# zju3dv/PVO

Hardware: AMD Instinct MI355X
Metric: VO keyframe updates/sec (8-keyframe window, 512x384, 36 edges; 6 graph updates + edge rebuild per keyframe) (higher is better)
Workload: dtype f16 (volume, lookup, update operator) / f32 (BA assembly) / f64 (pose solve); 1 GPU; S-B: BASELINE.json configs[1] window (8 keyframes, 48x64 maps, E=36, itrs=2), synthetic; edges=36, parallelism=independent window per GPU

## Files before the change

### pvo_amd/csrc/ba.hip

```cpp
#include "se3.h"
#include "conv1x1_tile.h"
#include "glo_tile.h"
#include <stdlib.h>
#include <type_traits>

namespace {

constexpr float kMinDepth = 0.25f;

constexpr double kFix = 268435456.0, kInvFix = 1.0 / 268435456.0;
__device__ __forceinline__ void fix_add(long long* sys, long long idx, double v, int* meta) {
  if (!(fabs(v) < 3.0e10)) { meta[4] = 1; return; }
#ifdef PVO_BA_NO_ATOMICS
  if (idx >= 0) return;
#endif
  atomicAdd(reinterpret_cast<unsigned long long*>(sys + idx), static_cast<unsigned long long>(__double2ll_rn(v * kFix)));
}
constexpr int kDealEdges = 2;
constexpr int kPPT = 2;
constexpr int kChunkA = 256 * kPPT;
constexpr int kMaxSep = 12;
constexpr int kXchgDoubles = 2 + 36 * kMaxSep * kMaxSep + 12 * kMaxSep;


// ... 2365 lines not shown
        const int ta0 = on0 ? 16 * tti[K] + lc - c0 : 0, tb0 = on0 ? 16 * ttj[K] + lc - c0 : 0;
        const int ta1 = on1 ? 16 * tti[K1] + lc - c0 : 0, tb1 = on1 ? 16 * ttj[K1] + lc - c0 : 0;
        double a00 = pan[dense_swz(ta0, lr)], b00 = pan[dense_swz(tb0, lr)], a01 = pan[dense_swz(ta0, 4 + lr)], b01 = pan[dense_swz(tb0, 4 + lr)];
        double a10 = pan[dense_swz(ta1, lr)], b10 = pan[dense_swz(tb1, lr)], a11 = pan[dense_swz(ta1, 4 + lr)], b11 = pan[dense_swz(tb1, 4 + lr)];
        if (!on0) { a00 = 0.0; a01 = 0.0; }
        if (!on1) { a10 = 0.0; a11 = 0.0; }
        C[K] = __builtin_amdgcn_mfma_f64_16x16x4f64(-a00, b00, C[K], 0, 0, 0);
        if (K + 1 < SLOTS) C[K1] = __builtin_amdgcn_mfma_f64_16x16x4f64(-a10, b10, C[K1], 0, 0, 0);
        C[K] = __builtin_amdgcn_mfma_f64_16x16x4f64(-a01, b01, C[K], 0, 0, 0);
        if (K + 1 < SLOTS) C[K1] = __builtin_amdgcn_mfma_f64_16x16x4f64(-a11, b11, C[K1], 0, 0, 0);
      };
      switch (u0 >> 1) {
#define PVO_DENSE_PAIR(K) case K / 2: if (K < SLOTS) { if (K >= nsl) break; pair(std::integral_constant<int, (K < SLOTS ? K : 0)>{}); } [[fallthrough]];
        PVO_DENSE_PAIR(0) PVO_DENSE_PAIR(2) PVO_DENSE_PAIR(4) PVO_DENSE_PAIR(6) PVO_DENSE_PAIR(8) PVO_DENSE_PAIR(10) PVO_DENSE_PAIR(12)
        PVO_DENSE_PAIR(14) PVO_DENSE_PAIR(16)
#undef PVO_DENSE_PAIR
        default: break;
      }
    }
    DENSE_STEP_PROBE(11);
    if (kb8 + 1 < nb) extract(kb8 + 1);
    DENSE_STEP_PROBE(12);
    DENSE_STEP_PROBE(13);
    __syncthreads();
    DENSE_STEP_PROBE(14);
  }
  BA_PROBE(2);

  if (wave == 0) {
    double z[3];
#pragma unroll
    for (int m = 0; m < 3; ++m) {
      const int c = lane + 64 * m;
      z[m] = c < n ? Lp[8 * dense_panel_off(c >> 3, N) + dense_swz(n - 8 * (c >> 3), c & 7)] : 0.0;
    }
    for (int kb8 = nb - 1; kb8 >= 0; --kb8) {
      const int c0 = 8 * kb8, m0 = c0 >> 6, l0 = c0 & 63;
      const int nv = (n - c0 < 8) ? n - c0 : 8;
      const double* pan = Lp + 8 * dense_panel_off(kb8, N);
      double Lk[28], rdv[8];
#pragma unroll
      for (int j = 0; j < 8; ++j) {
        rdv[j] = rdg[c0 + j];
#pragma unroll
        for (int i = j + 1; i < 8; ++i) Lk[i * (i - 1) / 2 + j] = pan[dense_swz(i, j)];
      }
      const double zsel = m0 == 0 ? z[0] : (m0 == 1 ? z[1] : z[2]);
      double x[8];
#pragma unroll
      for (int j = 0; j < 8; ++j) {
        const int lo = __builtin_amdgcn_readlane(static_cast<int>(__double_as_longlong(zsel) & 0xffffffffLL), l0 + j);
        const int hi = __builtin_amdgcn_readlane(static_cast<int>(__double_as_longlong(zsel) >> 32), l0 + j);
        x[j] = __longlong_as_double((static_cast<long long>(hi) << 32) | static_cast<unsigned int>(lo));
      }
#pragma unroll
      for (int j = 7; j >= 0; --j) {
        double v = x[j];
#pragma unroll
        for (int i = 7; i > j; --i) v -= Lk[i * (i - 1) / 2 + j] * x[i];
        x[j] = (j < nv) ? v * rdv[j] : 0.0;
      }
#pragma unroll
      for (int m = 0; m < 3; ++m) {
        const int c = lane + 64 * m;
        if (c < c0) {
          const double* pc = Lp + 8 * dense_panel_off(c >> 3, N);
          double v = z[m];
#pragma unroll
          for (int i = 0; i < 8; ++i) v -= pc[dense_swz(c0 + i - 8 * (c >> 3), c & 7)] * x[i];
          z[m] = v;
        } else if (c < c0 + 8) {
          double v = x[0];
#pragma unroll
          for (int j = 1; j < 8; ++j) v = (c - c0 == j) ? x[j] : v;
          z[m] = v;
        }
      }
    }
#pragma unroll
    for (int m = 0; m < 3; ++m) {
      const int c = lane + 64 * m;
      if (c < n) xs[c] = z[m];
    }
  }
  __syncthreads();
  BA_PROBE(4);
  solve_epilogue([&](int i) { return xs[i]; }, fail | meta[4] | meta[2], true, 0, P, t0, poses, dx_ws, dx_out, meta, status_out, true,
                 [] { BA_PROBE(5); });
}

constexpr int kNB = 48;
__global__ __launch_bounds__(256) void dense_panel_kernel(double* __restrict__ A, double* __restrict__ Ldiag, int n, int kb, int* __restrict__ meta) {
  __shared__ double Lk[kNB][kNB + 1];
  __shared__ double Xs[kNB][kNB + 1];
  __shared__ double rinv[kNB], ldg[kNB];
  const int tid = threadIdx.x;
  const int c0 = kNB * kb, nc = (n - c0 < kNB) ? n - c0 : kNB;
  const int rb = kb + blockIdx.x, r0 = kNB * rb;
  for (int t = tid; t < kNB * kNB; t += 256) {
    const int r = t / kNB, c = t - r * kNB;
    Lk[r][c] = (r < nc && c <= r) ? A[static_cast<size_t>(c0 + r) * n + c0 + c] : 0.0;
    const int rr = r0 + r;
    Xs[r][c] = (rr <= n && c < nc) ? A[static_cast<size_t>(rr) * n + c0 + c] : 0.0;
  }
  __syncthreads();
  bool ok = true;
  for (int j0 = 0; j0 < nc; j0 += 8) {
    const int nv = (nc - j0 < 8) ? nc - j0 : 8;
    double L[36], av[8];
    if (tid < 2 * kNB) {
      const bool isx = tid >= kNB;
      const int t = isx ? tid - kNB : tid;
      if (isx || (t >= j0 && t < nc)) {
        double (*Row)[kNB + 1] = isx ? Xs : Lk;
#pragma unroll
        for (int i = 0; i < 8; ++i) {
#pragma unroll
          for (int j = 0; j <= i; ++j) L[i * (i + 1) / 2 + j] = Lk[j0 + i][j0 + j];
        }
#pragma unroll
        for (int j = 0; j < 8; ++j) av[j] = Row[t][j0 + j];
      }
    }
    __syncthreads();
    if (tid < 2 * kNB) {
      const bool isx = tid >= kNB;
      const int t = isx ? tid - kNB : tid;
      if (isx || (t >= j0 && t < nc)) {
        double (*Row)[kNB + 1] = isx ? Xs : Lk;
#pragma unroll
        for (int j = 0; j < 8; ++j) {
          double d = L[j * (j + 1) / 2 + j];
#pragma unroll
          for (int k = 0; k < j; ++k) d -= L[j * (j + 1) / 2 + k] * L[j * (j + 1) / 2 + k];
          const bool real = j < nv;
          ok = ok && (!real || d > 0.0);
          const double rs = (real && ok) ? rsqrt_nr(d) : 0.0;
          if (!isx && t == j0 + j) { rinv[j0 + j] = rs; ldg[j0 + j] = d * rs; }
          L[j * (j + 1) / 2 + j] = rs;
#pragma unroll
          for (int i = j + 1; i < 8; ++i) {
            double v = L[i * (i + 1) / 2 + j];
#pragma unroll
            for (int k = 0; k < j; ++k) v -= L[i * (i + 1) / 2 + k] * L[j * (j + 1) / 2 + k];
            L[i * (i + 1) / 2 + j] = v * rs;
          }
          double v = av[j];
#pragma unroll
          for (int k = 0; k < j; ++k) v -= av[k] * L[j * (j + 1) / 2 + k];
          av[j] = v * rs;
        }
#pragma unroll
        for (int j = 0; j < 8; ++j) if (j < nv && (isx || j0 + j <= t)) Row[t][j0 + j] = av[j];
      }
    }
    __syncthreads();
    const int c1 = j0 + 8;
    if (c1 < nc) {
      const int ty = tid >> 4, tx = tid & 15;
      for (int r = c1 + ty; r < nc + kNB; r += 16) {
        const bool isx = r >= nc;
        double (*Row)[kNB + 1] = isx ? Xs : Lk;
        const int rr = isx ? r - nc : r;
        double a8[8];
#pragma unroll
        for (int k = 0; k < 8; ++k) a8[k] = Row[rr][j0 + k];
// ... 899 lines not shown
      hipLaunchKernelGGL(ba_schur_reduce_kernel, dim3(kSchurStagePairs, Kgrid), dim3(256), 0, st, w.plan, w.spart, w.srow, w.sT, sys, gx, 6 * P);
      PVO_CHECK_LAUNCH();
    }
  }
  return PVO_OK;
}

extern "C" int pvo_ba_finish(float* poses, float* disps, void* sys_,
                             const int64_t* ii, const int64_t* jj,
                             int E, int nframes, int ht, int wd, int t0, int t1,
                             float lm, float ep, int motion_only, int clamp_frames, float disp_min,
                             float* dx_out, float* dz_out, int dz_rows, int* status_out,
                             void* workspace, size_t workspace_bytes, void* stream) {
  return pvo_ba_finish_riders(poses, disps, sys_, ii, jj, E, nframes, ht, wd, t0, t1, lm, ep, motion_only, clamp_frames, disp_min,
                              dx_out, dz_out, dz_rows, status_out, workspace, workspace_bytes, nullptr, stream);
}

extern "C" int pvo_ba_finish_conv1x1(float* poses, float* disps, void* sys_,
                                     const int64_t* ii, const int64_t* jj,
                                     int E, int nframes, int ht, int wd, int t0, int t1,
                                     float lm, float ep, int motion_only, int clamp_frames, float disp_min,
                                     float* dx_out, float* dz_out, int dz_rows, int* status_out,
                                     void* workspace, size_t workspace_bytes,
                                     const void* cx, const void* cw, const float* cbias, void* cy, long long crows, int cCout, int cdtype,
                                     void* stream) {
  pvo_ba_riders r{};
  r.cx = cx; r.cw = cw; r.cbias = cbias; r.cy = cy; r.crows = crows; r.cCout = cCout; r.cdtype = cdtype;
  return pvo_ba_finish_riders(poses, disps, sys_, ii, jj, E, nframes, ht, wd, t0, t1, lm, ep, motion_only, clamp_frames, disp_min,
                              dx_out, dz_out, dz_rows, status_out, workspace, workspace_bytes, cy ? &r : nullptr, stream);
}

static int ba_finish_impl(float* poses, float* disps, void* sys_, const long long* msg, const int* first_s,
                          const int64_t* ii, const int64_t* jj,
                          int E, int nframes, int ht, int wd, int t0, int t1,
                          float lm, float ep, int motion_only, int clamp_frames, float disp_min,
                          float* dx_out, float* dz_out, int dz_rows, int* status_out,
                          void* workspace, size_t workspace_bytes,
                          const pvo_ba_riders* jobs, void* stream);

extern "C" int pvo_ba_finish_riders(float* poses, float* disps, void* sys_,
                                    const int64_t* ii, const int64_t* jj,
                                    int E, int nframes, int ht, int wd, int t0, int t1,
                                    float lm, float ep, int motion_only, int clamp_frames, float disp_min,
                                    float* dx_out, float* dz_out, int dz_rows, int* status_out,
                                    void* workspace, size_t workspace_bytes,
                                    const pvo_ba_riders* jobs, void* stream) {
  if (!sys_) return PVO_EINVAL;
  return ba_finish_impl(poses, disps, sys_, nullptr, nullptr, ii, jj, E, nframes, ht, wd, t0, t1, lm, ep, motion_only, clamp_frames, disp_min,
                        dx_out, dz_out, dz_rows, status_out, workspace, workspace_bytes, jobs, stream);
}

extern "C" size_t pvo_ba_packed_elems(const int* first_host, int P) {
  if (!first_host || P < 0) return 0;
  size_t blocks = 0;
  for (int b = 0; b < P; ++b) {
    const int f = first_host[b] < b ? (first_host[b] < 0 ? 0 : first_host[b]) : b;
    blocks += static_cast<size_t>(b - f + 1) * 36;
  }
  return blocks + static_cast<size_t>(6) * P;
}

extern "C" int pvo_ba_pack(void* sys_, const int* first_s, void* msg, int P, void* stream) {
  if (!sys_ || !first_s || !msg || P < 0) return PVO_EINVAL;
  if (P > kMaxEnvBlocks) return PVO_EUNSUPPORTED;
  if (P == 0) return PVO_OK;
  const int n6 = 6 * P;
  hipLaunchKernelGGL(ba_pack_kernel, dim3((n6 * n6 + n6 + 2047) / 2048), dim3(256), 0, pvo_stream(stream),
                     static_cast<long long*>(sys_), first_s, static_cast<long long*>(msg), n6);
  PVO_CHECK_LAUNCH();
  return PVO_OK;
}

extern "C" int pvo_ba_finish_packed(float* poses, float* disps, const void* msg, const int* first_s,
                                    const int64_t* ii, const int64_t* jj,
                                    int E, int nframes, int ht, int wd, int t0, int t1,
                                    float lm, float ep, int motion_only, int clamp_frames, float disp_min,
                                    float* dx_out, float* dz_out, int dz_rows, int* status_out,
                                    void* workspace, size_t workspace_bytes, void* stream) {
  if (!msg || !first_s) return PVO_EINVAL;
  return ba_finish_impl(poses, disps, nullptr, static_cast<const long long*>(msg), first_s, ii, jj, E, nframes, ht, wd, t0, t1, lm, ep, motion_only,
                        clamp_frames, disp_min, dx_out, dz_out, dz_rows, status_out, workspace, workspace_bytes, nullptr, stream);
}

enum SolveKind { kSolveStatus, kSolveDense, kSolveEnvelope, kSolveChain, kSolveBlocks };
struct SolveForm { SolveKind kind; int chol; };
static SolveForm solve_form(int P, int E, bool packed, int knob) {
  if (P == 0) return {kSolveStatus, 0};
  if (knob >= 1 && knob <= 3) return {kSolveChain, knob - 1};
  if (knob == 4) return {kSolveEnvelope, 2};
  if (knob == 6 && !packed) return {kSolveBlocks, 0};
  if (P <= kDenseMaxPoses) return {kSolveDense, 0};
  if (knob != 5 && !packed && static_cast<long long>(E) > 8LL * P) return {kSolveBlocks, 0};
  return {kSolveEnvelope, 2};
}

static int ba_finish_impl(float* poses, float* disps, void* sys_, const long long* msg, const int* first_s,
                          const int64_t* ii, const int64_t* jj,
                          int E, int nframes, int ht, int wd, int t0, int t1,
                          float lm, float ep, int motion_only, int clamp_frames, float disp_min,
                          float* dx_out, float* dz_out, int dz_rows, int* status_out,
                          void* workspace, size_t workspace_bytes,
                          const pvo_ba_riders* jobs, void* stream) {
  Riders rider{};
  size_t rider_lds = 0;
  if (jobs && jobs->cy && jobs->crows > 0) {
    if (!jobs->cx || !jobs->cw || jobs->cCout <= 0 || jobs->cCout % 192) return PVO_EINVAL;
    if (jobs->cdtype != PVO_F16 && jobs->cdtype != PVO_BF16) return PVO_EUNSUPPORTED;
    if (pvo_misaligned16(jobs->cx, jobs->cw, jobs->cy)) return PVO_EINVAL;
    if (jobs->crows > (1LL << 24)) return PVO_EUNSUPPORTED;
    rider.cx = static_cast<const uint16_t*>(jobs->cx); rider.cw = static_cast<const uint16_t*>(jobs->cw); rider.cbias = jobs->cbias;
    rider.cy = static_cast<uint16_t*>(jobs->cy); rider.crows = jobs->crows; rider.cCout = jobs->cCout; rider.cdtype = jobs->cdtype;
    rider.crow_blocks = static_cast<int>((jobs->crows + 63) / 64);
    rider.cblocks = rider.crow_blocks * (jobs->cCout / 192);
    rider_lds = c1t::kTileBytes;
  }
  if (jobs && jobs->gpart && jobs->gE > 0 && jobs->gHW > 0) {
    if (!jobs->gnet || !jobs->gw || jobs->gE > 65535) return PVO_EINVAL;
    if (jobs->gdtype != PVO_F16 && jobs->gdtype != PVO_BF16) return PVO_EUNSUPPORTED;
    if (pvo_misaligned16(jobs->gnet, jobs->gw)) return PVO_EINVAL;
    rider.gnet = static_cast<const uint16_t*>(jobs->gnet); rider.gw = static_cast<const uint16_t*>(jobs->gw); rider.gbias = jobs->gbias;
    rider.gpart = jobs->gpart; rider.gHW = jobs->gHW; rider.gchunks = (jobs->gHW + 255) / 256; rider.gdtype = jobs->gdtype;
    rider.gblocks = jobs->gE * rider.gchunks;
    if (rider_lds < static_cast<size_t>(glt::kTileBytes)) rider_lds = glt::kTileBytes;
  }
  if (jobs && jobs->xg && jobs->xE > 0) {
    if (!jobs->xpart || !jobs->xwt || !jobs->xbias || jobs->xchunks <= 0) return PVO_EINVAL;
    rider.xpart = jobs->xpart; rider.xwt = jobs->xwt; rider.xbias = jobs->xbias; rider.xg = jobs->xg;
    rider.xchunks = jobs->xchunks; rider.xblocks = jobs->xE;
    if (rider_lds < 512) rider_lds = 512;
  }
  const int rider_blocks = rider.cblocks + rider.gblocks + rider.xblocks;
  int rc = check_common(E, nframes, ht, wd, t0, t1);
  if (rc != PVO_OK) return rc;
  if (clamp_frames < 0 || clamp_frames > nframes) return PVO_EINVAL;
  const int P = t1 - t0, HW = ht * wd;
  long long* sys = static_cast<long long*>(sys_);
  if (!poses || !disps || (!sys && !msg) || !workspace) return PVO_EINVAL;
  if (P > kMaxEnvBlocks) return PVO_EUNSUPPORTED;
  if (workspace_bytes < pvo_ba_workspace_bytes(E, P, nframes, HW)) return PVO_EWORKSPACE;
  Ws w = carve(ws_base(workspace), E, P, nframes, HW);
  hipStream_t st = pvo_stream(stream);
  const int n6 = 6 * P;
  const SolveForm form = solve_form(P, E, msg != nullptr, pvo_knob(PVO_KNOB_BA_SOLVER));
  if (msg && form.kind == kSolveStatus) return PVO_OK;
  constexpr size_t kSolveLdsMax = 142000;
  if (form.kind == kSolveDense) {
    const size_t dl = dense_lds_bytes(n6);
    const size_t lds = dl > rider_lds ? dl : rider_lds;
    const int Td = dense_N(n6) / 16;
    if (!pvo_allow_lds<ba_solve_dense_kernel<4>>(kSolveLdsMax) || !pvo_allow_lds<ba_solve_dense_kernel<14>>(kSolveLdsMax) ||
        !pvo_allow_lds<ba_solve_dense_kernel<17>>(kSolveLdsMax))
      return PVO_ELAUNCH;
    const auto kernel = Td <= 5 ? ba_solve_dense_kernel<4> : (Td <= 10 ? ba_solve_dense_kernel<14> : ba_solve_dense_kernel<17>);
    hipLaunchKernelGGL(kernel, dim3(1 + rider_blocks), dim3(256), lds, st, sys, msg, first_s, poses, w.dx, dx_out, w.plan.meta, status_out,
                       P, t0, lm, ep, rider);
  } else if (form.kind == kSolveEnvelope || form.kind == kSolveChain) {
    int* part = form.kind == kSolveEnvelope ? reinterpret_cast<int*>(w.xchg) : nullptr;
    if (msg) {
      hipLaunchKernelGGL(ba_env_packed_kernel, dim3(P), dim3(256), 0, st, msg, first_s, w.plan.env, n6);
      hipLaunchKernelGGL(ba_prepare_packed_kernel, dim3(P + 1), dim3(256), 0, st, msg, first_s, w.chol, w.plan.env, n6, lm, ep,
                         static_cast<long long>(kSolveLdsMax), part);
    } else {
      hipLaunchKernelGGL(ba_env_kernel, dim3((n6 * n6 + 2047) / 2048), dim3(256), 0, st, sys, w.plan.env, n6);
      hipLaunchKernelGGL(ba_prepare_kernel, dim3((n6 * n6 + n6 + 2047) / 2048), dim3(256), 0, st, sys, w.chol, w.plan.env, n6, lm, ep,
                         static_cast<long long>(kSolveLdsMax), part);
    }
    PVO_CHECK_LAUNCH();
    if (!part && hipMemsetAsync(w.xchg, 0, 16, st) != hipSuccess) return PVO_ELAUNCH;
    if (!pvo_allow_lds<ba_solve_twin_kernel>(kSolveLdsMax)) return PVO_ELAUNCH;
    hipLaunchKernelGGL(ba_solve_twin_kernel, dim3(2 + rider_blocks), dim3(256), kSolveLdsMax > rider_lds ? kSolveLdsMax : rider_lds, st,
                       w.chol, poses, w.dx, dx_out, w.plan.meta, status_out, P, t0, w.plan.env, static_cast<long long>(kSolveLdsMax), w.xchg,
                       form.chol, rider);
  } else {
    if (form.kind == kSolveBlocks) {
      hipLaunchKernelGGL(ba_prepare_kernel, dim3((n6 * n6 + n6 + 2047) / 2048), dim3(256), 0, st, sys, w.chol, w.plan.env, n6, lm, ep,
                         0LL , static_cast<int*>(nullptr));
      PVO_CHECK_LAUNCH();
      if (hipMemsetAsync(w.xchg, 0, 16, st) != hipSuccess) return PVO_ELAUNCH;
      const int nkb = (n6 + kNB - 1) / kNB, nrb = (n6 + 1 + kNB - 1) / kNB;
      for (int kb = 0; kb < nkb; ++kb) {
        hipLaunchKernelGGL(dense_panel_kernel, dim3(nrb - kb), dim3(256), 0, st, w.chol, w.ldiag, n6, kb, w.plan.meta);
        const int m = nrb - kb - 1;
        if (m > 0) hipLaunchKernelGGL(dense_update_kernel, dim3(m * (m + 1) / 2), dim3(256), 0, st, w.chol, n6, kb, nrb);
      }
      PVO_CHECK_LAUNCH();
      double* yrow = w.chol + static_cast<size_t>(n6) * n6;
      for (int kb = nkb - 1; kb >= 0; --kb)
        hipLaunchKernelGGL(dense_back_kernel, dim3(kb + 1), dim3(256), 0, st, w.chol, w.ldiag, yrow, w.xvec, n6, kb);
      PVO_CHECK_LAUNCH();
    }
    if (rider_lds > 48 * 1024 && !pvo_allow_lds<dense_finish_kernel>(kSolveLdsMax)) return PVO_ELAUNCH;
    hipLaunchKernelGGL(dense_finish_kernel, dim3(1 + rider_blocks), dim3(256), rider_lds, st, w.xvec, poses, w.dx, dx_out, w.plan.meta, status_out, P, t0, rider);
  }
  PVO_CHECK_LAUNCH();
  if (!motion_only && E + P > 0) {
    const int Kmax = (nframes < P + E) ? nframes : (P + E);
    hipLaunchKernelGGL(ba_backsub_kernel, dim3((HW + 255) / 256, Kmax > clamp_frames ? Kmax : clamp_frames), dim3(256), 0, st,
                       w.plan, jj, w.Ei, w.Eij, w.Q, w.w, w.dx, disps, dz_out, dz_rows, HW, t0, P, clamp_frames, disp_min);
    PVO_CHECK_LAUNCH();
  }
  return PVO_OK;
}

extern "C" int pvo_ba_last_partition(void* workspace, size_t workspace_bytes, int E, int P, int nframes, int HW, int* out, void* stream) {
  if (!workspace || !out || E < 0 || P < 0) return PVO_EINVAL;
  if (workspace_bytes < pvo_ba_workspace_bytes(E, P, nframes, HW)) return PVO_EWORKSPACE;
  out[0] = out[1] = 0;
  const SolveKind kind = solve_form(P, E, false, pvo_knob(PVO_KNOB_BA_SOLVER)).kind;
  if (kind == kSolveStatus || kind == kSolveDense) return PVO_OK;
  Ws w = carve(ws_base(workspace), E, P, nframes, HW);
  int host[4] = {0, 0, 0, 0};
  if (hipMemcpyAsync(host, w.xchg, sizeof(host), hipMemcpyDeviceToHost, pvo_stream(stream)) != hipSuccess) return PVO_ELAUNCH;
  if (hipStreamSynchronize(pvo_stream(stream)) != hipSuccess) return PVO_ELAUNCH;
  out[0] = host[2]; out[1] = host[3];
  return PVO_OK;
}

extern "C" int pvo_ba_rig(float* poses, float* disps, const float* intrinsics,
                          const float* targets, const float* weights, const float* eta,
                          const int64_t* ii, const int64_t* jj,
                          int E, int nframes, int ht, int wd, int K_eta,
                          int t0, int t1, int iterations, float lm, float ep, int motion_only,
                          float* dx_out, float* dz_out, int dz_rows, int* status_out,
                          void* workspace, size_t workspace_bytes,
                          const float* disps_sens, float alpha, float baseline, void* stream) {
  int rc = check_common(E, nframes, ht, wd, t0, t1);
  if (rc != PVO_OK) return rc;
  if (iterations < 0) return PVO_EINVAL;
  if (disps_sens && !(alpha > 0.0f)) return PVO_EINVAL;
  if (!(baseline >= 0.0f) || !(baseline < __builtin_inff())) return PVO_EINVAL;
  const int P = t1 - t0, HW = ht * wd;
  if (!workspace) return PVO_EINVAL;
  if (workspace_bytes < pvo_ba_workspace_bytes(E, P, nframes, HW)) return PVO_EWORKSPACE;
  Ws w = carve(ws_base(workspace), E, P, nframes, HW);
  hipStream_t st = pvo_stream(stream);
  hipLaunchKernelGGL(ba_plan_kernel, dim3(1), dim3(256), 0, st, ii, jj, w.plan, E, nframes, t0, t1,
                     K_eta, motion_only, disps_sens, alpha, baseline);
  PVO_CHECK_LAUNCH();
  for (int it = 0; it < iterations; ++it) {
    rc = pvo_ba_local(poses, disps, intrinsics, targets, weights, eta, ii, jj, E, nframes, ht, wd, K_eta,
                      t0, t1, (motion_only ? 1 : 0) | (it > 0 ? 2 : 0), w.sys, workspace, workspace_bytes, stream);
    if (rc != PVO_OK) return rc;
    rc = pvo_ba_finish(poses, disps, w.sys, ii, jj, E, nframes, ht, wd, t0, t1, lm, ep, motion_only, 0, 0.0f,
                       dx_out, dz_out, dz_rows, status_out, workspace, workspace_bytes, stream);
    if (rc != PVO_OK) return rc;
  }
  return PVO_OK;
}

extern "C" int pvo_ba_prior(float* poses, float* disps, const float* intrinsics,
                            const float* targets, const float* weights, const float* eta,
                            const int64_t* ii, const int64_t* jj,
                            int E, int nframes, int ht, int wd, int K_eta,
                            int t0, int t1, int iterations, float lm, float ep, int motion_only,
                            float* dx_out, float* dz_out, int dz_rows, int* status_out,
                            void* workspace, size_t workspace_bytes,
                            const float* disps_sens, float alpha, void* stream) {
  return pvo_ba_rig(poses, disps, intrinsics, targets, weights, eta, ii, jj, E, nframes, ht, wd, K_eta, t0, t1, iterations, lm, ep,
                    motion_only, dx_out, dz_out, dz_rows, status_out, workspace, workspace_bytes, disps_sens, alpha, 0.0f, stream);
}

extern "C" int pvo_ba(float* poses, float* disps, const float* intrinsics,
                      const float* targets, const float* weights, const float* eta,
                      const int64_t* ii, const int64_t* jj,
                      int E, int nframes, int ht, int wd, int K_eta,
                      int t0, int t1, int iterations, float lm, float ep, int motion_only,
                      float* dx_out, float* dz_out, int dz_rows, int* status_out,
                      void* workspace, size_t workspace_bytes, void* stream) {
  return pvo_ba_prior(poses, disps, intrinsics, targets, weights, eta, ii, jj, E, nframes, ht, wd, K_eta, t0, t1, iterations, lm, ep,
                      motion_only, dx_out, dz_out, dz_rows, status_out, workspace, workspace_bytes, nullptr, 0.0f, stream);
}

extern "C" int pvo_ba_sigma(const void* sys_, void* workspace, size_t workspace_bytes,
                            const int64_t* ii, const int64_t* jj,
                            int E, int P, int nframes, int ht, int wd, int t0, float lm, float ep,
                            double* pose_cov, float* var_cond, float* var_pose, int* status_out, void* stream) {
  if (P < 0) return PVO_EINVAL;
  int rc = check_common(E, nframes, ht, wd, t0, t0 + P);
  if (rc != PVO_OK) return rc;
  if (P > kSigmaMaxPoses) return PVO_EUNSUPPORTED;
  if (!workspace || (P > 0 && (!sys_ || !pose_cov))) return PVO_EINVAL;
  if (E == 0 || !ii || !jj) return PVO_EINVAL;
  const int HW = ht * wd, n = 6 * P;
  if (workspace_bytes < pvo_ba_workspace_bytes(E, P, nframes, HW)) return PVO_EWORKSPACE;
  Ws w = carve(ws_base(workspace), E, P, nframes, HW);
  hipStream_t st = pvo_stream(stream);
  if (P > 0) {
    hipLaunchKernelGGL(ba_sigma_prepare_kernel, dim3((n * n + 255) / 256), dim3(256), 0, st, static_cast<const long long*>(sys_), w.chol, n, lm, ep);
    hipLaunchKernelGGL(ba_sigma_factor_kernel, dim3(1), dim3(1024), 0, st, w.chol, n, w.plan.meta, status_out);
    hipLaunchKernelGGL(ba_sigma_invtri_kernel, dim3(n), dim3(64), 0, st, w.chol, n);
    hipLaunchKernelGGL(ba_sigma_product_kernel, dim3((n + 63) / 64, n), dim3(64), 0, st, w.chol, pose_cov, n);
    PVO_CHECK_LAUNCH();
// ... 91 lines not shown
```

### pvo_amd/droid_backends.py

```python
import ctypes
import itertools

import torch

from . import _lib
from ._lib import PvoHipError, check

_DT = {torch.float32: _lib.PVO_F32, torch.float16: _lib.PVO_F16,
       torch.bfloat16: _lib.PVO_BF16, torch.float64: _lib.PVO_F64}

_ws_cache = {}


def _contig(t, name):
    if not t.is_contiguous():
        raise RuntimeError("%s must be contiguous" % name)


def _dev(*ts):
    dev = None
    for t in ts:
        if t is None:
            continue
        if not t.is_cuda:
# ... 1333 lines not shown
    stride = int(stride)
    y = torch.empty(N, Cout, (H - 1) // stride + 1, (W - 1) // stride + 1, dtype=x.dtype, device=dev)
    with torch.cuda.device(dev):
        check(_lib.load().pvo_conv1x1_planes(_ptr(x), _ptr(w), _vp(bias), _ptr(y), N, Cin, Cout, H, W, stride, _dtype_code(x, "x"), _stream(dev)), "conv1x1_planes")
    return y


def conv_planes_supported(ksize, stride, cin, cout):
    return bool(_lib.load().pvo_conv_planes_supported(int(ksize), int(stride), int(cin), int(cout)))


class PackedConvFilter:
    __slots__ = ("frag", "ksize", "cin", "cout", "dtype")

    def __init__(self, frag, ksize, cin, cout, dtype):
        self.frag, self.ksize, self.cin, self.cout, self.dtype = frag, ksize, cin, cout, dtype


def conv_planes_pack(weight):
    dev = _dev(weight)
    if weight.dim() != 4 or weight.shape[2] != weight.shape[3] or weight.dtype not in (torch.float16, torch.bfloat16) or not weight.is_contiguous():
        raise PvoHipError("conv_planes_pack: weight must be a contiguous 16-bit [Cout,Cin,k,k] tensor")
    Cout, Cin, k, _ = weight.shape
    lib = _lib.load()
    nbytes = lib.pvo_conv_planes_filter_bytes(k, Cin, Cout)
    if nbytes == 0:
        raise PvoHipError("conv_planes_pack: unsupported filter %d x %d, %d -> %d channels" % (k, k, Cin, Cout))
    frag = torch.empty(nbytes // 2, dtype=weight.dtype, device=dev)
    with torch.cuda.device(dev):
        check(lib.pvo_conv_planes_pack(_ptr(weight), _ptr(frag), k, Cin, Cout, _dtype_code(weight, "weight"), _stream(dev)), "conv_planes_pack")
    return PackedConvFilter(frag, k, Cin, Cout, weight.dtype)


def conv_planes(x, packed, bias=None, residual=None, stride=1, relu_inner=False, relu_outer=False, out=None):
    if not isinstance(packed, PackedConvFilter):
        raise PvoHipError("conv_planes: packed must come from conv_planes_pack")
    dev = _dev(x, packed.frag, bias, residual, out)
    if x.dim() != 4 or x.dtype not in (torch.float16, torch.bfloat16) or not x.is_contiguous():
        raise PvoHipError("conv_planes: x must be a contiguous 16-bit [N,Cin,H,W] tensor")
    N, Cin, H, W = x.shape
    stride = int(stride)
    if packed.dtype != x.dtype or packed.cin != Cin:
        raise PvoHipError("conv_planes: the packed filter is %s with %d input channels, x is %s with %d" % (packed.dtype, packed.cin, x.dtype, Cin))
    Cout, k = packed.cout, packed.ksize
    if stride < 1 or not conv_planes_supported(k, stride, Cin, Cout):
        raise PvoHipError("conv_planes: unsupported convolution %d x %d stride %d, %d -> %d channels" % (k, k, stride, Cin, Cout))
    shape = (N, Cout, (H - 1) // stride + 1 if H else 0, (W - 1) // stride + 1 if W else 0)
    for t, n in ((bias, "bias"), (residual, "residual"), (out, "out")):
        if t is not None and (t.dtype != x.dtype or not t.is_contiguous()):
            raise PvoHipError("conv_planes: %s must be contiguous and have x's dtype" % n)
    if bias is not None and bias.numel() != Cout or residual is not None and tuple(residual.shape) != shape \
            or out is not None and tuple(out.shape) != shape:
        raise PvoHipError("conv_planes: bias [Cout], residual and out of the result's shape %s" % (shape,))
    if out is not None and out.numel() and x.numel() and out.untyped_storage().data_ptr() == x.untyped_storage().data_ptr() \
            and out.data_ptr() < x.data_ptr() + x.numel() * 2 and x.data_ptr() < out.data_ptr() + out.numel() * 2:
        raise PvoHipError("conv_planes: out must not alias x")
    y = torch.empty(shape, dtype=x.dtype, device=dev) if out is None else out
    with torch.cuda.device(dev):
        check(_lib.load().pvo_conv_planes(_ptr(x), _ptr(packed.frag), _vp(bias), _vp(residual), _ptr(y), N, Cin, Cout, H, W, k, stride,
                                          1 if relu_inner else 0, 1 if relu_outer else 0, _dtype_code(x, "x"), _stream(dev)), "conv_planes")
    return y


_FRAME_KINDS = {torch.int32: 0, torch.uint8: 1, torch.float32: 2}


def frame_normalise(image, mean, std, dtype=torch.float16):
    dev = _dev(image)
    _contig(image, "image")
    if image.dim() != 3 or image.shape[0] != 3 or image.dtype not in _FRAME_KINDS:
        raise PvoHipError("frame_normalise: a contiguous [3,H,W] int32 / uint8 / float32 frame")
    _, H, W = image.shape
    out = torch.empty(1, 3, H, W, dtype=dtype, device=dev)
    m = (ctypes.c_float * 3)(*[float(v) for v in mean]); s = (ctypes.c_float * 3)(*[float(v) for v in std])
    with torch.cuda.device(dev):
        check(_lib.load().pvo_frame_normalise(_ptr(image), _ptr(out), H, W, m, s, _FRAME_KINDS[image.dtype], _DT[dtype], _stream(dev)), "frame_normalise")
    return out


def debug_config(knob, value):
    knobs = {"ba_solver": _lib.PVO_KNOB_BA_SOLVER, "heads_gather_flat": _lib.PVO_KNOB_HEADS_GATHER_FLAT, "no_riders": _lib.PVO_KNOB_NO_RIDERS,
             "post_separate": _lib.PVO_KNOB_POST_SEPARATE}
    if knob == "ba_solver":
        value = {None: 0, "": 0, "blocked": 1, "wave": 2, "pipe": 3, "twin": 4, "dense": 5, "blocks": 6}[value]
    check(_lib.load().pvo_debug_config(knobs[knob], int(value)), "pvo_debug_config")


def graph_update_workspace(E, K, R, H, W, max_segments, device):
    n = _lib.load().pvo_graph_update_workspace_bytes(int(E), int(K), int(R), int(H), int(W), int(max_segments))
    return _op_workspace(("up", torch.device(device).index), torch.device(device), n)


def graph_update(weights, args, workspace, stereo_baseline=0.0):
    dev = workspace.device
    stereo_baseline = _baseline(stereo_baseline, "graph_update")
    with torch.cuda.device(dev):
        if stereo_baseline == 0.0:
            check(_lib.load().pvo_graph_update(ctypes.byref(weights.struct), ctypes.byref(args), ctypes.c_void_p(workspace.data_ptr()),
                                               workspace.numel(), _stream(dev)), "graph_update")
        else:
            check(_lib.load().pvo_graph_update_rig(ctypes.byref(weights.struct), ctypes.byref(args), ctypes.c_void_p(workspace.data_ptr()),
                                                   workspace.numel(), stereo_baseline, _stream(dev)), "graph_update (stereo)")


def _cvx_mask_layout(mask, what):
    if mask.dim() != 4 or mask.shape[1] != 576:
        raise PvoHipError("%s: mask must be [B,576,H,W] (9 taps x 8 x 8 logits); got %s" % (what, tuple(mask.shape)))
    if mask.is_contiguous():
        return 1
    if mask.permute(0, 2, 3, 1).is_contiguous():
        return 0
    raise RuntimeError("mask must be contiguous")


def _cvx_rows(rows, B, n, dev, name):
    if rows is None:
        return None
    if not isinstance(rows, torch.Tensor):
        rows = [int(r) for r in rows]
        if any(r < 0 or r >= n for r in rows):
            raise PvoHipError("cvx_upsample: %s names a row outside the buffer of %d rows" % (name, n))
        rows = to_device_async(rows, torch.long, dev)
    _dev(rows); _long(rows, name); _contig(rows, name)
    if rows.dim() != 1 or rows.shape[0] != B:
        raise PvoHipError("cvx_upsample: %s must have one entry per mask row (%d)" % (name, B))
    return rows


def cvx_upsample(data, mask, out=None, in_rows=None, out_rows=None):
    dev = _dev(data, mask, out)
    _contig(data, "data")
    planar = _cvx_mask_layout(mask, "cvx_upsample")
    if data.dim() != 4 or data.shape[3] not in (1, 2) or tuple(data.shape[1:3]) != tuple(mask.shape[2:]):
        raise PvoHipError("cvx_upsample: data must be [N,H,W,D] with D = 1 or 2 and the mask's H, W; got %s for mask %s"
                          % (tuple(data.shape), tuple(mask.shape)))
    B, _, H, W = mask.shape
    N, D = data.shape[0], data.shape[3]
    if out is None:
        out = torch.empty(B if out_rows is None else N, 8 * H, 8 * W, D, dtype=data.dtype, device=dev)
    _contig(out, "out")
    if out.dim() != 4 or tuple(out.shape[1:]) != (8 * H, 8 * W, D) or out.dtype != data.dtype:
        raise PvoHipError("cvx_upsample: out must be [N',%d,%d,%d] %s" % (8 * H, 8 * W, D, data.dtype))
    if (in_rows is None and N < B) or (out_rows is None and out.shape[0] < B):
        raise PvoHipError("cvx_upsample: %d mask rows need %d rows of data and out (or row tables)" % (B, B))
    in_rows = _cvx_rows(in_rows, B, N, dev, "in_rows")
    out_rows = _cvx_rows(out_rows, B, out.shape[0], dev, "out_rows")
    with torch.cuda.device(dev):
        check(_lib.load().pvo_cvx_upsample(_ptr(data), _ptr(mask), _ptr(out), _vp(in_rows), _vp(out_rows), N, out.shape[0], B, H, W, D,
                                           mask.shape[1], planar, _dtype_code(data, "cvx_upsample"), _dtype_code(mask, "cvx_upsample"),
                                           _stream(dev)), "cvx_upsample")
    return out


def cvx_upsample_vjp(data, mask, gout):
    dev = _dev(data, mask, gout)
    _contig(data, "data"); _contig(gout, "gout")
    planar = _cvx_mask_layout(mask, "cvx_upsample_vjp")
    B, _, H, W = mask.shape
    D = data.shape[-1]
    if tuple(data.shape) != (B, H, W, D) or tuple(gout.shape) != (B, 8 * H, 8 * W, D) or not (data.dtype == mask.dtype == gout.dtype) \
            or data.dtype not in (torch.float32, torch.float64):
        raise PvoHipError("cvx_upsample_vjp: data [B,H,W,D], mask [B,576,H,W], gout [B,8H,8W,D], all fp32 or all fp64")
    gmask, gdata = torch.empty_like(mask), torch.empty_like(data)
    lib = _lib.load()
    dt = _DT[data.dtype]
    scratch = torch.empty(lib.pvo_cvx_upsample_vjp_scratch_bytes(B, H, W, D, dt), dtype=torch.uint8, device=dev)
    with torch.cuda.device(dev):
# ... 220 lines not shown
```

Measured before the change: 249.9 keyframe updates/s.

## Add register-resident single-wave Cholesky solver for small pose windows

```diff
diff --git a/pvo_amd/csrc/ba.hip b/pvo_amd/csrc/ba.hip
--- a/pvo_amd/csrc/ba.hip
+++ b/pvo_amd/csrc/ba.hip
@@ -2471,6 +2471,135 @@
       const int c = lane + 64 * m;
       if (c < n) xs[c] = z[m];
     }
+  }
+  __syncthreads();
+  BA_PROBE(4);
+  solve_epilogue([&](int i) { return xs[i]; }, fail | meta[4] | meta[2], true, 0, P, t0, poses, dx_ws, dx_out, meta, status_out, true,
+                 [] { BA_PROBE(5); });
+}
+
+constexpr int kSmallMaxPoses = 10;
+__host__ __device__ constexpr int small_pitch(int n) { return n | 1; }
+__host__ constexpr size_t small_lds_bytes(int n) { return 16 + sizeof(double) * (64 * static_cast<size_t>(small_pitch(n)) + 64); }
+
+__device__ __forceinline__ double readlane_f64(double v, int src) {
+  const int lo = __builtin_amdgcn_readlane(static_cast<int>(__double_as_longlong(v) & 0xffffffffLL), src);
+  const int hi = __builtin_amdgcn_readlane(static_cast<int>(__double_as_longlong(v) >> 32), src);
+  return __longlong_as_double((static_cast<long long>(hi) << 32) | static_cast<unsigned int>(lo));
+}
+
+template <class F, int... J>
+__device__ __forceinline__ void static_for(F&& f, std::integer_sequence<int, J...>) { (f(std::integral_constant<int, J>{}), ...); }
+
+template <int P>
+__global__ __launch_bounds__(256) __attribute__((amdgpu_waves_per_eu(2, 2))) void ba_solve_small_kernel(
+    long long* __restrict__ sys, const long long* __restrict__ msg, const int* __restrict__ first_s,
+    float* __restrict__ poses, float* __restrict__ dx_ws, float* __restrict__ dx_out,
+    int* __restrict__ meta, int* __restrict__ status_out, int t0, float lm, float ep, Riders riders) {
+  extern __shared__ __attribute__((aligned(16))) unsigned char smem[];
+  if (blockIdx.x > 0) {
+    ride(smem, riders, blockIdx.x - 1);
+    return;
+  }
+  constexpr int n = 6 * P, RP = small_pitch(n), TOT = (n + 1) * n, PER = (TOT + 255) / 256;
+  __shared__ int mfirst[kSmallMaxPoses + 1], mbase[kSmallMaxPoses + 2];
+  if (msg) {
+    if (threadIdx.x == 0) {
+      int run = 0;
+      for (int b = 0; b < P; ++b) {
+        const int e = first_s[b];
+        const int f = e < b ? (e < 0 ? 0 : e) : b;
+        mfirst[b] = f; mbase[b] = run; run += (b - f + 1) * 36;
+      }
+      mbase[P] = run;
+    }
+    __syncthreads();
+  }
+  int& fail = *reinterpret_cast<int*>(smem);
+  double* Lr = reinterpret_cast<double*>(smem + 16);
+  double* xs = Lr + 64 * RP;
+  const int tid = threadIdx.x, lane = tid & 63, wave = __builtin_amdgcn_readfirstlane(tid >> 6);
+  BA_PROBE(0);
+#ifdef PVO_BA_PROBE
+  if (g_ba_probe && tid == 0) g_ba_probe[15] = 0x5A11;
+#endif
+  auto load = [&](auto from_message) {
+    constexpr bool MSG = decltype(from_message)::value;
+    const long long* __restrict__ src = MSG ? msg : sys;
+    long long raw[PER];
+#pragma unroll
+    for (int u = 0; u < PER; ++u) {
+      const int e = tid + 256 * u, row = e / n, col = e - row * n;
+      int idx = -1;
+      if (MSG) {
+        const int rw = row < n ? row : 0;
+        const int rb = rw / 6, cb = col / 6;
+        const int body = mbase[rb] + (cb - mfirst[rb]) * 36 + (rw - 6 * rb) * 6 + (col - 6 * cb);
+        idx = (row < n && col <= row && cb >= mfirst[rb]) ? body : (row == n ? mbase[P] + col : -1);
+      } else {
+        idx = (row < n && col <= row) ? row * n + col : (row == n ? n * n + col : -1);
+      }
+      const long long v = src[idx < 0 ? 0 : idx];
+      raw[u] = idx < 0 ? 0LL : v;
+    }
+#pragma unroll
+    for (int u = 0; u < PER; ++u) {
+      const int e = tid + 256 * u, row = e / n, col = e - row * n;
+      double v = static_cast<double>(raw[u]) * kInvFix;
+      if (row == col) v += static_cast<double>(ep) + static_cast<double>(lm) * v;
+      if (e < TOT) Lr[row * RP + col] = v;
+    }
+  };
+  if (msg) load(std::true_type{}); else load(std::false_type{});
+  __syncthreads();
+  BA_PROBE(1);
+  if (wave != 0) {
+    if (!msg) for (int idx = tid - 64; idx < n * n + n; idx += 192) sys[idx] = 0LL;
+  } else {
+    double a[n];
+#pragma unroll
+    for (int c = 0; c < n; ++c) {
+      const double v = Lr[lane * RP + c];
+      a[c] = lane <= n ? v : 0.0;
+    }
+    wave_lds_sync();
+    bool ok = true;
+    double myrs = 0.0;
+    static_for([&](auto jc) {
+      constexpr int j = decltype(jc)::value;
+      const double d = readlane_f64(a[j], j);
+      ok = ok && d > 0.0;
+      const double rs = ok ? rsqrt_nr1(d) : 0.0;
+      const double l = lane > j ? a[j] * rs : 0.0;
+      myrs = lane == j ? rs : myrs;
+      Lr[lane * RP + j] = l;
+      if (j + 1 < n) a[j + 1] -= l * readlane_f64(l, j + 1);
+      wave_lds_sync();
+      constexpr int kChunk = 32;
+#pragma unroll
+      for (int k0 = j + 2; k0 < n; k0 += kChunk) {
+        double m[kChunk];
+#pragma unroll
+        for (int u = 0; u < kChunk; ++u)
+          if (k0 + u < n) m[u] = Lr[(k0 + u) * RP + j];
+        asm volatile("" ::: "memory");
+#pragma unroll
+        for (int u = 0; u < kChunk; ++u)
+          if (k0 + u < n) a[k0 + u] -= l * m[u];
+      }
+    }, std::make_integer_sequence<int, n>{});
+    BA_PROBE(2);
+    double z = lane < n ? Lr[n * RP + lane] : 0.0;
+    double Lj[n];
+#pragma unroll
+    for (int j = 0; j < n; ++j) {
+      const double v = Lr[j * RP + lane];
+      Lj[j] = lane < j ? v : 0.0;
+    }
+#pragma unroll
+    for (int j = n - 1; j >= 0; --j) z -= Lj[j] * readlane_f64(z * myrs, j);
+    if (lane < n) xs[lane] = z * myrs;
+    if (lane == 0) fail = ok ? 0 : 1;
   }
   __syncthreads();
   BA_PROBE(4);
@@ -3536,13 +3665,14 @@
                         clamp_frames, disp_min, dx_out, dz_out, dz_rows, status_out, workspace, workspace_bytes, nullptr, stream);
 }
 
-enum SolveKind { kSolveStatus, kSolveDense, kSolveEnvelope, kSolveChain, kSolveBlocks };
+enum SolveKind { kSolveStatus, kSolveSmall, kSolveDense, kSolveEnvelope, kSolveChain, kSolveBlocks };
 struct SolveForm { SolveKind kind; int chol; };
 static SolveForm solve_form(int P, int E, bool packed, int knob) {
   if (P == 0) return {kSolveStatus, 0};
   if (knob >= 1 && knob <= 3) return {kSolveChain, knob - 1};
   if (knob == 4) return {kSolveEnvelope, 2};
   if (knob == 6 && !packed) return {kSolveBlocks, 0};
+  if (knob != 5 && P <= kSmallMaxPoses) return {kSolveSmall, 0};
   if (P <= kDenseMaxPoses) return {kSolveDense, 0};
   if (knob != 5 && !packed && static_cast<long long>(E) > 8LL * P) return {kSolveBlocks, 0};
   return {kSolveEnvelope, 2};
@@ -3598,7 +3728,21 @@
   const SolveForm form = solve_form(P, E, msg != nullptr, pvo_knob(PVO_KNOB_BA_SOLVER));
   if (msg && form.kind == kSolveStatus) return PVO_OK;
   constexpr size_t kSolveLdsMax = 142000;
-  if (form.kind == kSolveDense) {
+  if (form.kind == kSolveSmall) {
+    const size_t sl = small_lds_bytes(n6);
+    const size_t lds = sl > rider_lds ? sl : rider_lds;
+    switch (P) {
+#define PVO_SMALL_CASE(N) case N: \
+      if (lds > 48 * 1024 && !pvo_allow_lds<ba_solve_small_kernel<N>>(kSolveLdsMax)) return PVO_ELAUNCH; \
+      hipLaunchKernelGGL(ba_solve_small_kernel<N>, dim3(1 + rider_blocks), dim3(256), lds, st, sys, msg, first_s, poses, w.dx, dx_out, \
+                         w.plan.meta, status_out, t0, lm, ep, rider); \
+      break;
+      PVO_SMALL_CASE(1) PVO_SMALL_CASE(2) PVO_SMALL_CASE(3) PVO_SMALL_CASE(4) PVO_SMALL_CASE(5) PVO_SMALL_CASE(6) PVO_SMALL_CASE(7)
+      PVO_SMALL_CASE(8) PVO_SMALL_CASE(9) PVO_SMALL_CASE(10)
+#undef PVO_SMALL_CASE
+      default: return PVO_EINVAL;
+    }
+  } else if (form.kind == kSolveDense) {
     const size_t dl = dense_lds_bytes(n6);
     const size_t lds = dl > rider_lds ? dl : rider_lds;
     const int Td = dense_N(n6) / 16;
@@ -3661,7 +3805,7 @@
   if (workspace_bytes < pvo_ba_workspace_bytes(E, P, nframes, HW)) return PVO_EWORKSPACE;
   out[0] = out[1] = 0;
   const SolveKind kind = solve_form(P, E, false, pvo_knob(PVO_KNOB_BA_SOLVER)).kind;
-  if (kind == kSolveStatus || kind == kSolveDense) return PVO_OK;
+  if (kind == kSolveStatus || kind == kSolveSmall || kind == kSolveDense) return PVO_OK;
   Ws w = carve(ws_base(workspace), E, P, nframes, HW);
   int host[4] = {0, 0, 0, 0};
   if (hipMemcpyAsync(host, w.xchg, sizeof(host), hipMemcpyDeviceToHost, pvo_stream(stream)) != hipSuccess) return PVO_ELAUNCH;
diff --git a/pvo_amd/droid_backends.py b/pvo_amd/droid_backends.py
--- a/pvo_amd/droid_backends.py
+++ b/pvo_amd/droid_backends.py
@@ -1439,7 +1439,7 @@
     knobs = {"ba_solver": _lib.PVO_KNOB_BA_SOLVER, "heads_gather_flat": _lib.PVO_KNOB_HEADS_GATHER_FLAT, "no_riders": _lib.PVO_KNOB_NO_RIDERS,
              "post_separate": _lib.PVO_KNOB_POST_SEPARATE}
     if knob == "ba_solver":
-        value = {None: 0, "": 0, "blocked": 1, "wave": 2, "pipe": 3, "twin": 4, "dense": 5, "blocks": 6}[value]
+        value = {None: 0, "": 0, "blocked": 1, "wave": 2, "pipe": 3, "twin": 4, "dense": 5, "blocks": 6, "small": 7}[value]
     check(_lib.load().pvo_debug_config(knobs[knob], int(value)), "pvo_debug_config")
 
 
```

Result: no change. 251.9 keyframe updates/s, median of 6 (+0.8%).
